# zyc-123/InstanceDiff

Measured on AMD Instinct MI355X. Metric: denoising steps/sec (256x256 bs16), higher is better.
Workload: dtype f32; 1 GPU; 256x256 1-ch synthetic, 1000-step reverse chain, batch 16 per GPU, 2 UNet fwd + reverse update per step; global_batch=16, parallelism=replicas x1 (no collective)

## Files before the change

### instancediff_amd/csrc/attention.hip

```cpp
#include <math.h>
#include <type_traits>
#include <stdlib.h>

#include "common.h"

namespace {

#define KAPPA(r) (((r) & 3) + 8 * ((r) >> 2))

template <int DH>
__global__ __launch_bounds__(256) void attn_self_kernel(const float* __restrict__ qkv, float* __restrict__ out, float* __restrict__ lse, int C,
                                                        int N, int heads, float scale) {
    constexpr int MB = DH / 32;
    constexpr int KT = DH * 32;
    constexpr int VT = DH * 33;
    constexpr int BUF = KT + VT + 3;
    constexpr int NV4 = DH * 32 / 4 / 256;
    extern __shared__ __attribute__((aligned(16))) float smem[];

    const int tid = threadIdx.x, lane = tid & 63, wave = tid >> 6, half = lane >> 5, l31 = lane & 31;
    const int b = blockIdx.y / heads, h = blockIdx.y % heads;
    const int q0 = (blockIdx.x * 4 + wave) * 32;
    const float* qb = qkv + (long long)b * 3 * C * N + (long long)(h * DH) * N;
    const float* kb = qb + (long long)C * N;
    const float* vb = qb + (long long)2 * C * N;

    float qreg[DH / 2];
    const int qi = q0 + l31;
#pragma unroll
    for (int s = 0; s < DH / 2; ++s) qreg[s] = qi < N ? qb[(long long)(2 * s + half) * N + qi] : 0.f;

    floatx16 O[MB];
#pragma unroll
    for (int m = 0; m < MB; ++m)
#pragma unroll
        for (int r = 0; r < 16; ++r) O[m][r] = 0.f;
    float mrun = -INFINITY, lrun = 0.f;

    const int nkb = (N + 31) / 32;
    floatx4 rk[NV4], rv[NV4];
    auto load_tile = [&](int kbi) {
        const int key0 = kbi * 32;
#pragma unroll
        for (int i = 0; i < NV4; ++i) {
            const int f = tid + i * 256;
            const int d = f >> 3, j4 = (f & 7) * 4;
            floatx4 kz = {0.f, 0.f, 0.f, 0.f}, vz = {0.f, 0.f, 0.f, 0.f};
            if (key0 + j4 + 3 < N) {
                kz = *reinterpret_cast<const floatx4*>(kb + (long long)d * N + key0 + j4);
                vz = *reinterpret_cast<const floatx4*>(vb + (long long)d * N + key0 + j4);
            } else {
                for (int e = 0; e < 4; ++e)
                    if (key0 + j4 + e < N) {
                        kz[e] = kb[(long long)d * N + key0 + j4 + e];
                        vz[e] = vb[(long long)d * N + key0 + j4 + e];
                    }
            }
            rk[i] = kz;
            rv[i] = vz;
        }
    };
    auto write_tile = [&](int buf) {
        float* kt = smem + buf * BUF;
        float* vt = kt + KT;
#pragma unroll
        for (int i = 0; i < NV4; ++i) {
            const int f = tid + i * 256;
            const int d = f >> 3, j4 = (f & 7) * 4;
#pragma unroll
            for (int e = 0; e < 4; ++e) {
                kt[d * 32 + j4 + e] = rk[i][e];
                vt[d * 33 + j4 + e] = rv[i][e];
            }
        }
    };

    load_tile(0);
    write_tile(0);
    __syncthreads();
    for (int kbi = 0; kbi < nkb; ++kbi) {
        const int buf = kbi & 1;
        if (kbi + 1 < nkb) load_tile(kbi + 1);
        const float* kt = smem + buf * BUF;
        const float* vt = kt + KT;
        floatx16 S;
#pragma unroll
        for (int r = 0; r < 16; ++r) S[r] = 0.f;
#pragma unroll
        for (int s = 0; s < DH / 2; ++s) S = __builtin_amdgcn_mfma_f32_32x32x2f32(kt[(2 * s + half) * 32 + l31], qreg[s], S, 0, 0, 0);
// ... 398 lines not shown
#pragma unroll
        for (int i = 0; i < NF4; ++i) {
            const int f = lane + i * 64;
            const int c = f >> 3, j4 = (f & 7) * 4;
            if (XCW % 8 != 0 && f >= XCW * 8) continue;
#pragma unroll
            for (int e = 0; e < 4; ++e) tile[c * 33 + j4 + e] = rt[i][e];
        }
    };

    if (kb_begin < kb_end) {
        load_tile(kb_begin);
        write_tile();
    }
    for (int kbi = kb_begin; kbi < kb_end; ++kbi) {
        if (kbi + 1 < kb_end) load_tile(kbi + 1);
        floatx16 S;
#pragma unroll
        for (int r = 0; r < 16; ++r) S[r] = 0.f;
#pragma unroll
        for (int t = 0; t < XCW / 2; ++t) S = __builtin_amdgcn_mfma_f32_32x32x2f32(tile[(2 * t + half) * 33 + l31], qreg[t], S, 0, 0, 0);
#pragma unroll
        for (int r = 0; r < 16; ++r) xch[(wave * 16 + r) * 64 + lane] = S[r];
        __syncthreads();
        const int key0 = kbi * 32 + 4 * half;
        float mx = -INFINITY;
#pragma unroll
        for (int r = 0; r < 16; ++r) {
            float sv = xch[(0 * 16 + r) * 64 + lane] + xch[(1 * 16 + r) * 64 + lane] + xch[(2 * 16 + r) * 64 + lane] + xch[(3 * 16 + r) * 64 + lane];
            sv = (key0 + KAPPA(r) < N) ? sv * scale : -INFINITY;
            S[r] = sv;
            mx = fmaxf(mx, sv);
        }
        mx = fmaxf(mx, __shfl_xor(mx, 32, 64));
        const float mnew = fmaxf(mrun, mx);
        const float alpha = __expf(mrun - mnew);
        float ps = 0.f;
#pragma unroll
        for (int r = 0; r < 16; ++r) {
            const float p = __expf(S[r] - mnew);
            S[r] = p;
            ps += p;
        }
        lrun = lrun * alpha + ps;
        mrun = mnew;
        if (__any(alpha != 1.f)) {
#pragma unroll
            for (int m = 0; m < XCB; ++m)
#pragma unroll
                for (int r = 0; r < 16; ++r) O[m][r] *= alpha;
        }
#pragma unroll
        for (int r = 0; r < 16; ++r)
#pragma unroll
            for (int m = 0; m < XCB; ++m)
                O[m] = __builtin_amdgcn_mfma_f32_32x32x2f32(tile[(m * 32 + l31) * 33 + KAPPA(r) + 4 * half], S[r], O[m], 0, 0, 0);
        if (kbi + 1 < kb_end) write_tile();
        __syncthreads();
    }
    float* wp = ws + ((long long)b * nsplit + sp) * (XCM + 2) * 32;
    const float l = lrun + __shfl_xor(lrun, 32, 64);
#pragma unroll
    for (int m = 0; m < XCB; ++m)
#pragma unroll
        for (int r = 0; r < 16; ++r) {
            const int cl = m * 32 + KAPPA(r) + 4 * half;
            if (cl < XCW) wp[(c0 + cl) * 32 + l31] = O[m][r];
        }
    if (wave == 0 && half == 0) {
        wp[XCM * 32 + l31] = mrun;
        wp[(XCM + 1) * 32 + l31] = l;
    }
}
template <int XCW>
__global__ __launch_bounds__(256) void smm_xattn_kernel(const float* __restrict__ qf, const float* __restrict__ mem, float* __restrict__ ws,
                                                        int rows, int N, int nsplit, int kps, float scale) {
    smm_xattn_body<XCW>(qf, mem, ws, rows, N, nsplit, kps, scale, blockIdx.y, blockIdx.x);
}

template <int CM>
__device__ __forceinline__ void smm_xattn_w_body(const float* __restrict__ qf, const float* __restrict__ mem, float* __restrict__ ws, int rows, int N,
                                                 int nsplit, int kps, float scale, const int b, const int sp) {
    constexpr int CB = (CM + 31) / 32;
    constexpr int TILE = CB * 32 * 33;
    constexpr int NF4 = (CM * 8 + 63) / 64;
    extern __shared__ __attribute__((aligned(16))) float smem[];
    const int tid = threadIdx.x, lane = tid & 63, wave = tid >> 6, half = lane >> 5, l31 = lane & 31;
    float* tile = smem + wave * TILE;
    const float* memb = mem + (long long)b * CM * N;
    for (int i = lane; i < TILE; i += 64) tile[i] = 0.f;

    float qreg[CM / 2];
#pragma unroll
    for (int t = 0; t < CM / 2; ++t) qreg[t] = l31 < rows ? qf[((long long)b * rows + l31) * CM + 2 * t + half] : 0.f;
    floatx16 O[CB];
#pragma unroll
    for (int m = 0; m < CB; ++m)
#pragma unroll
        for (int r = 0; r < 16; ++r) O[m][r] = 0.f;
    float mrun = -INFINITY, lrun = 0.f;

    const int nkb = (N + 31) / 32;
    const int kb_begin = sp * kps + wave;
    const int kb_end = min(nkb, sp * kps + kps);
    floatx4 rt[NF4];
    auto load_tile = [&](int kbi) {
        const int key0 = kbi * 32;
#pragma unroll
        for (int i = 0; i < NF4; ++i) {
            const int f = lane + i * 64;
            const int c = f >> 3, j4 = (f & 7) * 4;
            floatx4 z = {0.f, 0.f, 0.f, 0.f};
            if ((CM * 8) % 64 != 0 && f >= CM * 8) {
            } else if (key0 + j4 + 3 < N)
                z = *reinterpret_cast<const floatx4*>(memb + (long long)c * N + key0 + j4);
            else
                for (int e = 0; e < 4; ++e)
                    if (key0 + j4 + e < N) z[e] = memb[(long long)c * N + key0 + j4 + e];
            rt[i] = z;
        }
    };
    auto write_tile = [&]() {
#pragma unroll
        for (int i = 0; i < NF4; ++i) {
            const int f = lane + i * 64;
            const int c = f >> 3, j4 = (f & 7) * 4;
            if ((CM * 8) % 64 != 0 && f >= CM * 8) continue;
#pragma unroll
            for (int e = 0; e < 4; ++e) tile[c * 33 + j4 + e] = rt[i][e];
        }
    };
    if (kb_begin < kb_end) load_tile(kb_begin);
    for (int kbi = kb_begin; kbi < kb_end; kbi += 4) {
        write_tile();
        if (kbi + 4 < kb_end) load_tile(kbi + 4);
        floatx16 S;
#pragma unroll
        for (int r = 0; r < 16; ++r) S[r] = 0.f;
#pragma unroll
        for (int t = 0; t < CM / 2; ++t) S = __builtin_amdgcn_mfma_f32_32x32x2f32(tile[(2 * t + half) * 33 + l31], qreg[t], S, 0, 0, 0);
        const int key0 = kbi * 32 + 4 * half;
        float mx = -INFINITY;
#pragma unroll
        for (int r = 0; r < 16; ++r) {
            const float sv = (key0 + KAPPA(r) < N) ? S[r] * scale : -INFINITY;
            S[r] = sv;
            mx = fmaxf(mx, sv);
        }
        mx = fmaxf(mx, __shfl_xor(mx, 32, 64));
        const float mnew = fmaxf(mrun, mx);
        const float alpha = __expf(mrun - mnew);
        float ps = 0.f;
#pragma unroll
        for (int r = 0; r < 16; ++r) {
            const float p = __expf(S[r] - mnew);
            S[r] = p;
            ps += p;
        }
        lrun = lrun * alpha + ps;
        mrun = mnew;
        if (__any(alpha != 1.f)) {
#pragma unroll
            for (int m = 0; m < CB; ++m)
#pragma unroll
                for (int r = 0; r < 16; ++r) O[m][r] *= alpha;
        }
#pragma unroll
        for (int r = 0; r < 16; ++r)
#pragma unroll
            for (int m = 0; m < CB; ++m)
                O[m] = __builtin_amdgcn_mfma_f32_32x32x2f32(tile[(m * 32 + l31) * 33 + KAPPA(r) + 4 * half], S[r], O[m], 0, 0, 0);
    }
    static_assert((CM + 2) * 32 <= TILE, "partial does not fit the tile area");
    const float l = lrun + __shfl_xor(lrun, 32, 64);
#pragma unroll
    for (int m = 0; m < CB; ++m)
#pragma unroll
        for (int r = 0; r < 16; ++r) {
            const int cl = m * 32 + KAPPA(r) + 4 * half;
            if (cl < CM) tile[cl * 32 + l31] = O[m][r];
        }
    if (half == 0) {
        tile[CM * 32 + l31] = mrun;
        tile[(CM + 1) * 32 + l31] = l;
    }
    __syncthreads();
    float* wp = ws + ((long long)b * nsplit + sp) * (CM + 2) * 32;
    for (int i = tid; i < CM * 32; i += 256) {
        const int row = i & 31;
        float M = -INFINITY;
#pragma unroll
        for (int w = 0; w < 4; ++w) M = fmaxf(M, smem[w * TILE + CM * 32 + row]);
        float acc = 0.f;
#pragma unroll
        for (int w = 0; w < 4; ++w) {
            const float ms = smem[w * TILE + CM * 32 + row];
            acc += smem[w * TILE + i] * (ms == -INFINITY ? 0.f : __expf(ms - M));
        }
        wp[i] = acc;
    }
    if (tid < 32) {
        float M = -INFINITY, L = 0.f;
#pragma unroll
        for (int w = 0; w < 4; ++w) M = fmaxf(M, smem[w * TILE + CM * 32 + tid]);
#pragma unroll
        for (int w = 0; w < 4; ++w) {
            const float ms = smem[w * TILE + CM * 32 + tid];
            L += smem[w * TILE + (CM + 1) * 32 + tid] * (ms == -INFINITY ? 0.f : __expf(ms - M));
        }
        wp[CM * 32 + tid] = M;
        wp[(CM + 1) * 32 + tid] = L;
    }
}
template <int CM>
__global__ __launch_bounds__(256) void smm_xattn_w_kernel(const float* __restrict__ qf, const float* __restrict__ mem, float* __restrict__ ws, int rows,
                                                          int N, int nsplit, int kps, float scale) {
    smm_xattn_w_body<CM>(qf, mem, ws, rows, N, nsplit, kps, scale, blockIdx.y, blockIdx.x);
}

constexpr int CSL = 4;
__device__ __forceinline__ void smm_xattn_combine_body(const float* __restrict__ ws, float* __restrict__ o, int rows, int nsplit, int XCM,
                                                       float* __restrict__ lse, const int b, const int bx) {
    __shared__ float red[3][CSL][64];
    const int io = threadIdx.x & 63, sl = threadIdx.x >> 6;
    const int i = bx * 64 + io;
    const int c = i >> 5, row = i & 31;
    const bool live = i < XCM * 32 && row < rows;
    const long long ss = (long long)(XCM + 2) * 32;
    const float* wb = ws + (long long)b * nsplit * ss;
    float M = -INFINITY, L = 0.f, acc = 0.f;
    if (live) {
#pragma unroll 8
        for (int s = sl; s < nsplit; s += CSL) M = fmaxf(M, wb[s * ss + XCM * 32 + row]);
#pragma unroll 8
        for (int s = sl; s < nsplit; s += CSL) {
            const float* w = wb + s * ss;
            const float ms = w[XCM * 32 + row];
            const float f = ms == -INFINITY ? 0.f : __expf(ms - M);
            L += w[(XCM + 1) * 32 + row] * f;
            acc += w[c * 32 + row] * f;
        }
    }
    red[0][sl][io] = M, red[1][sl][io] = L, red[2][sl][io] = acc;
    __syncthreads();
    if (sl == 0 && live) {
        float Mt = red[0][0][io];
#pragma unroll
        for (int l = 1; l < CSL; ++l) Mt = fmaxf(Mt, red[0][l][io]);
        float Lt = 0.f, At = 0.f;
#pragma unroll
        for (int l = 0; l < CSL; ++l) {
            const float ml = red[0][l][io];
            const float f = ml == -INFINITY ? 0.f : __expf(ml - Mt);
            Lt += red[1][l][io] * f;
            At += red[2][l][io] * f;
        }
        o[((long long)b * rows + row) * XCM + c] = At / Lt;
        if (lse && c == 0) lse[(long long)b * rows + row] = Mt + __logf(Lt);
    }
}
__global__ __launch_bounds__(256) void smm_xattn_combine_kernel(const float* __restrict__ ws, float* __restrict__ o, int rows, int nsplit, int XCM,
                                                                float* __restrict__ lse) {
    smm_xattn_combine_body(ws, o, rows, nsplit, XCM, lse, blockIdx.y, blockIdx.x);
}

struct XattnGroups {
    idiff_xattn_group g[IDIFF_XATTN_MAX_GROUPS];
    int nsplit[IDIFF_XATTN_MAX_GROUPS], kps[IDIFF_XATTN_MAX_GROUPS], kind[IDIFF_XATTN_MAX_GROUPS];
};
__global__ __launch_bounds__(256) __attribute__((amdgpu_waves_per_eu(2))) void smm_xattn_grouped_kernel(const XattnGroups args, int rows, float scale) {
    const int z = blockIdx.z;
    const idiff_xattn_group& d = args.g[z];
    const int ns = args.nsplit[z], kps = args.kps[z];
    if ((int)blockIdx.x >= ns) return;
    switch (args.kind[z]) {
        case 0: smm_xattn_body<64>(d.qf, d.mem, d.ws, rows, d.N, ns, kps, scale, blockIdx.y, blockIdx.x); break;
        case 1: smm_xattn_body<34>(d.qf, d.mem, d.ws, rows, d.N, ns, kps, scale, blockIdx.y, blockIdx.x); break;
        case 2: smm_xattn_body<18>(d.qf, d.mem, d.ws, rows, d.N, ns, kps, scale, blockIdx.y, blockIdx.x); break;
        default: smm_xattn_w_body<72>(d.qf, d.mem, d.ws, rows, d.N, ns, kps, scale, blockIdx.y, blockIdx.x); break;
    }
}
__global__ __launch_bounds__(256) void smm_xattn_combine_grouped_kernel(const XattnGroups args, int rows) {
    const int z = blockIdx.z;
    const idiff_xattn_group& d = args.g[z];
    if ((int)blockIdx.x * 64 >= d.Cm * 32) return;
    smm_xattn_combine_body(d.ws, d.o, rows, args.nsplit[z], d.Cm, nullptr, blockIdx.y, blockIdx.x);
}

template <int XCW>
__global__ __launch_bounds__(256) void smm_xattn_bwd_kernel(const float* __restrict__ qf, const float* __restrict__ mem, const float* __restrict__ o,
                                                            const float* __restrict__ lse, const float* __restrict__ d_o, float* __restrict__ ws,
                                                            float* __restrict__ dmem, int rows, int N, int nsplit, int kps, float scale,
                                                            int accumulate) {
    constexpr int XCM = 4 * XCW, XCB = (XCW + 31) / 32, XTILE = XCB * 32 * 33, XP = XCM + 1, XREG = 2304;
    constexpr int NF4 = (XCW * 8 + 63) / 64;
    extern __shared__ __attribute__((aligned(16))) float smem[];
    float* tile = smem + (threadIdx.x >> 6) * XTILE;
    float* qL = smem + 4 * XTILE;
// ... 243 lines not shown
    else if (dh == 32)
        hipLaunchKernelGGL(attn_ctx_kernel<32>, grid, dim3(256), lds, st, q, k, v, out, C, N, M, scale);
    else if (dh == 64)
        hipLaunchKernelGGL(attn_ctx_kernel<64>, grid, dim3(256), lds, st, q, k, v, out, C, N, M, scale);
    else
        IDIFF_FAIL(IDIFF_E_UNSUPPORTED, "attn_ctx: head dim must be 16, 32 or 64 (got %d)", dh);
    IDIFF_CHECK_LAUNCH("attn_ctx_fwd");
    return IDIFF_OK;
}

extern "C" int idiff_attn_tokens_fwd(const float* q, const float* k, const float* v, float* out, int B, int Nq, int M, int C, int heads,
                                     float scale, int64_t ldq, int64_t ldkv, idiff_stream_t stream) {
    IDIFF_CHECK_ARG(q && k && v && out && B > 0 && Nq > 0 && C > 0 && heads > 0 && C % heads == 0, "attn_tokens: bad args");
    IDIFF_CHECK_ARG(M >= 1 && M <= 64, "attn_tokens: M must be in 1..64 (got %d)", M);
    IDIFF_CHECK_ARG(ldq >= C && ldkv >= C, "attn_tokens: row strides must be >= C");
    hipLaunchKernelGGL(attn_tokens_kernel, dim3(B * heads * Nq), dim3(64), 0, (hipStream_t)stream, q, k, v, out, Nq, M, C, heads, scale,
                       (long long)ldq, (long long)ldkv);
    IDIFF_CHECK_LAUNCH("attn_tokens_fwd");
    return IDIFF_OK;
}

extern "C" int idiff_attn_tokens_bwd(const float* q, const float* k, const float* v, const float* d_o, float* dq, float* dk, float* dv, int B, int Nq,
                                     int M, int C, int heads, float scale, int64_t ldq, int64_t ldkv, int64_t ldo, int64_t lddq, int64_t lddkv,
                                     idiff_stream_t stream) {
    IDIFF_CHECK_ARG(q && k && v && d_o && dq && dk && dv && B > 0 && C > 0 && heads > 0 && C % heads == 0, "attn_tokens_bwd: bad args");
    IDIFF_CHECK_ARG(Nq >= 1 && Nq <= ATB && M >= 1 && M <= ATB, "attn_tokens_bwd: Nq and M must be in 1..%d (got %d, %d)", ATB, Nq, M);
    IDIFF_CHECK_ARG(C / heads <= 64, "attn_tokens_bwd: head dim must be <= 64 (got %d)", C / heads);
    IDIFF_CHECK_ARG(ldq >= C && ldkv >= C && ldo >= C && lddq >= C && lddkv >= C, "attn_tokens_bwd: row strides must be >= C");
    hipLaunchKernelGGL(attn_tokens_bwd_kernel, dim3(B * heads), dim3(64), 0, (hipStream_t)stream, q, k, v, d_o, dq, dk, dv, Nq, M, C, heads, scale,
                       (long long)ldq, (long long)ldkv, (long long)ldo, (long long)lddq, (long long)lddkv);
    IDIFF_CHECK_LAUNCH("attn_tokens_bwd");
    return IDIFF_OK;
}

extern "C" int idiff_attn_tokens_grouped_fwd(const float* const* q, const float* const* k, const float* const* v, float* const* out, int ngroups,
                                             int B, int Nq, int M, int C, int heads, float scale, int64_t ldq, int64_t ldkv, idiff_stream_t stream) {
    IDIFF_CHECK_ARG(q && k && v && out && ngroups >= 1 && ngroups <= IDIFF_LINEAR_MAX_GROUPS, "attn_tokens_grouped: 1..%d groups", IDIFF_LINEAR_MAX_GROUPS);
    IDIFF_CHECK_ARG(B > 0 && Nq > 0 && C > 0 && heads > 0 && C % heads == 0, "attn_tokens_grouped: bad args");
    IDIFF_CHECK_ARG(M >= 1 && M <= 64, "attn_tokens_grouped: M must be in 1..64 (got %d)", M);
    IDIFF_CHECK_ARG(ldq >= C && ldkv >= C, "attn_tokens_grouped: row strides must be >= C");
    AttnTokGroups g;
    memset(&g, 0, sizeof(g));
    for (int i = 0; i < ngroups; ++i) {
        IDIFF_CHECK_ARG(q[i] && k[i] && v[i] && out[i], "attn_tokens_grouped: group %d: null pointer", i);
        g.q[i] = q[i], g.k[i] = k[i], g.v[i] = v[i], g.out[i] = out[i];
    }
    hipLaunchKernelGGL(attn_tokens_grouped_kernel, dim3(B * heads * Nq, ngroups), dim3(64), 0, (hipStream_t)stream, g, Nq, M, C, heads, scale,
                       (long long)ldq, (long long)ldkv);
    IDIFF_CHECK_LAUNCH("attn_tokens_grouped_fwd");
    return IDIFF_OK;
}

extern "C" int64_t idiff_smm_xattn_ws_floats(int B, int Nq, int heads, int Cm, int N) {
    (void)Nq;
    (void)heads;
    int ns, kps;
    smm_split(B, N, &ns, &kps);
    return (int64_t)B * ns * (Cm + 2) * 32;
}

static int smm_xattn_fwd_impl(const float* qf, const float* mem, float* o, float* lse, float* ws, int B, int Nq, int heads, int Cm, int N, float scale,
                              idiff_stream_t stream) {
    IDIFF_CHECK_ARG(qf && mem && o && ws && B > 0 && Nq > 0 && heads > 0 && N > 0, "smm_xattn: bad args");
    IDIFF_CHECK_ARG(Cm == 256 || Cm == 136 || Cm == 72, "smm_xattn: Cm must be 72, 136 or 256 (got %d)", Cm);
    IDIFF_CHECK_ARG(Nq * heads <= 32, "smm_xattn: Nq*heads must be <= 32 (got %d)", Nq * heads);
    IDIFF_CHECK_ARG(N % 4 == 0, "smm_xattn: N must be a multiple of 4");
    int ns, kps;
    smm_split(B, N, &ns, &kps);
    const int rows = Nq * heads;
    hipStream_t st = (hipStream_t)stream;
    const int xcb = (Cm / 4 + 31) / 32;
    const size_t lds = (size_t)(4 * xcb * 32 * 33 + 4 * 16 * 64) * sizeof(float);
    int ns_eff = ns;
    if (Cm == 256)
        hipLaunchKernelGGL(smm_xattn_kernel<64>, dim3(ns, B), dim3(256), lds, st, qf, mem, ws, rows, N, ns, kps, scale);
    else if (Cm == 136)
        hipLaunchKernelGGL(smm_xattn_kernel<34>, dim3(ns, B), dim3(256), lds, st, qf, mem, ws, rows, N, ns, kps, scale);
    else if (kps >= 4) {
        static const bool wform_off = [] {
            const char* e = getenv("IDIFF_XATTN_WFORM");
            return e && e[0] == '0';
        }();
        if (!wform_off) {
            const size_t ldsw = (size_t)4 * 3 * 32 * 33 * sizeof(float);
            hipLaunchKernelGGL(smm_xattn_w_kernel<72>, dim3(ns, B), dim3(256), ldsw, st, qf, mem, ws, rows, N, ns, kps, scale);
        } else {
            hipLaunchKernelGGL(smm_xattn_kernel<18>, dim3(ns, B), dim3(256), lds, st, qf, mem, ws, rows, N, ns, kps, scale);
        }
    } else
        hipLaunchKernelGGL(smm_xattn_kernel<18>, dim3(ns, B), dim3(256), lds, st, qf, mem, ws, rows, N, ns, kps, scale);
    IDIFF_CHECK_LAUNCH("smm_xattn_fwd");
    hipLaunchKernelGGL(smm_xattn_combine_kernel, dim3((32 * Cm + 63) / 64, B), dim3(256), 0, st, ws, o, rows, ns_eff, Cm, lse);
    IDIFF_CHECK_LAUNCH("smm_xattn_combine");
    return IDIFF_OK;
}

extern "C" int idiff_smm_xattn_grouped_fwd(const idiff_xattn_group* groups, int ngroups, int B, int Nq, int heads, float scale, idiff_stream_t stream) {
    IDIFF_CHECK_ARG(groups && ngroups >= 1 && ngroups <= IDIFF_XATTN_MAX_GROUPS, "smm_xattn_grouped: 1..%d groups", IDIFF_XATTN_MAX_GROUPS);
    IDIFF_CHECK_ARG(B > 0 && Nq > 0 && heads > 0 && Nq * heads <= 32, "smm_xattn_grouped: Nq*heads must be in 1..32 (got %d)", Nq * heads);
    XattnGroups args;
    memset(&args, 0, sizeof(args));
    int gx = 0, gc = 0;
    size_t lds = 0;
    for (int i = 0; i < ngroups; ++i) {
        const idiff_xattn_group& d = groups[i];
        IDIFF_CHECK_ARG(d.qf && d.mem && d.o && d.ws && d.N > 0 && d.N % 4 == 0, "smm_xattn_grouped: group %d: bad args", i);
        IDIFF_CHECK_ARG(d.Cm == 256 || d.Cm == 136 || d.Cm == 72, "smm_xattn_grouped: group %d: Cm must be 72, 136 or 256 (got %d)", i, d.Cm);
        args.g[i] = d;
        smm_split(B, d.N, &args.nsplit[i], &args.kps[i]);
        const int xcb = (d.Cm / 4 + 31) / 32;
        size_t l = (size_t)(4 * xcb * 32 * 33 + 4 * 16 * 64) * sizeof(float);
        if (d.Cm == 256) args.kind[i] = 0;
        else if (d.Cm == 136) args.kind[i] = 1;
        else if (args.kps[i] >= 4) args.kind[i] = 3, l = (size_t)4 * 3 * 32 * 33 * sizeof(float);
        else args.kind[i] = 2;
        lds = max(lds, l);
        gx = max(gx, args.nsplit[i]);
        gc = max(gc, (32 * d.Cm + 63) / 64);
    }
    hipStream_t st = (hipStream_t)stream;
    hipLaunchKernelGGL(smm_xattn_grouped_kernel, dim3(gx, B, ngroups), dim3(256), lds, st, args, Nq * heads, scale);
    IDIFF_CHECK_LAUNCH("smm_xattn_grouped_fwd");
    hipLaunchKernelGGL(smm_xattn_combine_grouped_kernel, dim3(gc, B, ngroups), dim3(256), 0, st, args, Nq * heads);
    IDIFF_CHECK_LAUNCH("smm_xattn_grouped_combine");
    return IDIFF_OK;
}

extern "C" int idiff_smm_xattn_fwd(const float* qf, const float* mem, float* o, float* ws, int B, int Nq, int heads, int Cm, int N, float scale,
                                   idiff_stream_t stream) {
    return smm_xattn_fwd_impl(qf, mem, o, nullptr, ws, B, Nq, heads, Cm, N, scale, stream);
}

extern "C" int idiff_smm_xattn_lse_fwd(const float* qf, const float* mem, float* o, float* lse, float* ws, int B, int rows, int N, float scale,
                                       idiff_stream_t stream) {
    IDIFF_CHECK_ARG(lse, "smm_xattn_lse_fwd: null lse");
    return smm_xattn_fwd_impl(qf, mem, o, lse, ws, B, rows, 1, 256, N, scale, stream);
}

extern "C" int idiff_smm_xattn_cm_lse_fwd(const float* qf, const float* mem, float* o, float* lse, float* ws, int B, int rows, int Cm, int N,
                                          float scale, idiff_stream_t stream) {
    IDIFF_CHECK_ARG(lse, "smm_xattn_cm_lse_fwd: null lse");
    return smm_xattn_fwd_impl(qf, mem, o, lse, ws, B, rows, 1, Cm, N, scale, stream);
}

static int smm_xattn_bwd_impl(const float* qf, const float* mem, const float* o, const float* lse, const float* d_o, float* dqf, float* dmem,
                              int accumulate, float* ws, int B, int rows, int Cm, int N, float scale, idiff_stream_t stream) {
    IDIFF_CHECK_ARG(qf && mem && o && lse && d_o && dqf && dmem && ws && B > 0 && N > 0, "smm_xattn_bwd: bad args");
    IDIFF_CHECK_ARG(rows >= 1 && rows <= 32, "smm_xattn_bwd: rows must be in 1..32 (got %d)", rows);
    IDIFF_CHECK_ARG(Cm == 256 || Cm == 72, "smm_xattn_bwd: Cm must be 72 or 256 (got %d)", Cm);
    IDIFF_CHECK_ARG(N % 4 == 0, "smm_xattn_bwd: N must be a multiple of 4");
    int ns, kps;
    smm_split(B, N, &ns, &kps);
    hipStream_t st = (hipStream_t)stream;
    const int xcb = (Cm / 4 + 31) / 32;
    const size_t lds = (size_t)(4 * xcb * 32 * 33 + 2 * 32 * (Cm + 1) + 4 * 2304 + 64) * sizeof(float);
    static bool attr[2] = {false, false};
    const int which = Cm == 256 ? 0 : 1;
    if (!attr[which]) {
        hipError_t e = Cm == 256 ? hipFuncSetAttribute(reinterpret_cast<const void*>(smm_xattn_bwd_kernel<64>), hipFuncAttributeMaxDynamicSharedMemorySize, (int)lds)
                                 : hipFuncSetAttribute(reinterpret_cast<const void*>(smm_xattn_bwd_kernel<18>), hipFuncAttributeMaxDynamicSharedMemorySize, (int)lds);
        if (e != hipSuccess) IDIFF_FAIL(IDIFF_E_HIP, "smm_xattn_bwd: hipFuncSetAttribute: %s", hipGetErrorString(e));
        attr[which] = true;
    }
    if (Cm == 256)
        hipLaunchKernelGGL(smm_xattn_bwd_kernel<64>, dim3(ns, B), dim3(256), lds, st, qf, mem, o, lse, d_o, ws, dmem, rows, N, ns, kps, scale, accumulate);
    else
        hipLaunchKernelGGL(smm_xattn_bwd_kernel<18>, dim3(ns, B), dim3(256), lds, st, qf, mem, o, lse, d_o, ws, dmem, rows, N, ns, kps, scale, accumulate);
    IDIFF_CHECK_LAUNCH("smm_xattn_bwd");
    hipLaunchKernelGGL(smm_xattn_bwd_combine_kernel, dim3((Cm * 32 + 255) / 256, B), dim3(256), 0, st, ws, dqf, rows, ns, Cm);
    IDIFF_CHECK_LAUNCH("smm_xattn_bwd_combine");
    return IDIFF_OK;
}

extern "C" int idiff_smm_xattn_bwd(const float* qf, const float* mem, const float* o, const float* lse, const float* d_o, float* dqf, float* dmem,
                                   int accumulate, float* ws, int B, int rows, int N, float scale, idiff_stream_t stream) {
    return smm_xattn_bwd_impl(qf, mem, o, lse, d_o, dqf, dmem, accumulate, ws, B, rows, 256, N, scale, stream);
}

extern "C" int idiff_smm_xattn_cm_bwd(const float* qf, const float* mem, const float* o, const float* lse, const float* d_o, float* dqf, float* dmem,
                                      int accumulate, float* ws, int B, int rows, int Cm, int N, float scale, idiff_stream_t stream) {
    return smm_xattn_bwd_impl(qf, mem, o, lse, d_o, dqf, dmem, accumulate, ws, B, rows, Cm, N, scale, stream);
}
```

### instancediff_amd/csrc/conv1x1_x3.hip

```cpp
#include <stdlib.h>

#include <type_traits>

#include "conv_args.h"

using idiff_detail::ConvArgs;

namespace {

typedef unsigned uintx4 __attribute__((ext_vector_type(4)));
typedef __bf16 bf16x8 __attribute__((ext_vector_type(8)));

constexpr int BM = 64, CKB = 32, NT = 256;
constexpr int B_ISTR = 1088;
constexpr int B_KGSTR = 4 * B_ISTR;
constexpr int B_PLSTR = 4 * B_KGSTR;
constexpr int B_BYTES = 3 * B_PLSTR;
constexpr int A_PLSTR = 4 * 64 * 16;
constexpr int A_BYTES = 3 * A_PLSTR;
constexpr int OLD = 256 + 4;
static_assert(32 * OLD * 4 <= B_BYTES, "epilogue tile must fit in the B planes");

__host__ __device__ constexpr unsigned hi16(unsigned u) { return u & 0xffff0000u; }

__device__ __forceinline__ unsigned pack_hi(unsigned odd, unsigned even) { return __builtin_amdgcn_perm(odd, even, 0x07060302u); }

__device__ __forceinline__ void split3(const float (&x)[8], uintx4& p1, uintx4& p2, uintx4& p3) {
    unsigned u1[8], u2[8], u3[8];
#pragma unroll
    for (int c = 0; c < 8; ++c) {
        u1[c] = __builtin_bit_cast(unsigned, x[c]);
        const float r1 = x[c] - __builtin_bit_cast(float, hi16(u1[c]));
        u2[c] = __builtin_bit_cast(unsigned, r1);
        const float r2 = r1 - __builtin_bit_cast(float, hi16(u2[c]));
        u3[c] = __builtin_bit_cast(unsigned, r2);
    }
    p1 = uintx4{pack_hi(u1[1], u1[0]), pack_hi(u1[3], u1[2]), pack_hi(u1[5], u1[4]), pack_hi(u1[7], u1[6])};
    p2 = uintx4{pack_hi(u2[1], u2[0]), pack_hi(u2[3], u2[2]), pack_hi(u2[5], u2[4]), pack_hi(u2[7], u2[6])};
    p3 = uintx4{pack_hi(u3[1], u3[0]), pack_hi(u3[3], u3[2]), pack_hi(u3[5], u3[4]), pack_hi(u3[7], u3[6])};
}

template <typename T>
__device__ __forceinline__ T* scalar_ptr(const T* p) {
    const unsigned long long v = reinterpret_cast<unsigned long long>(p);
    const unsigned lo = __builtin_amdgcn_readfirstlane((unsigned)v), hi = __builtin_amdgcn_readfirstlane((unsigned)(v >> 32));
    return reinterpret_cast<T*>(((unsigned long long)hi << 32) | lo);
}

__device__ __forceinline__ floatx4 mma(const uintx4& a, const uintx4& b, const floatx4& c) {
    return __builtin_amdgcn_mfma_f32_16x16x32_bf16(__builtin_bit_cast(bf16x8, a), __builtin_bit_cast(bf16x8, b), c, 0, 0, 0);
}

template <bool UNSH>
__global__ __launch_bounds__(NT) __attribute__((amdgpu_waves_per_eu(2, 2))) void conv1x1_x3_kernel(const ConvArgs a, const unsigned short* __restrict__ wx3) {
    extern __shared__ __attribute__((aligned(16))) unsigned char smem_raw[];
    unsigned char* const Bs = smem_raw;
    unsigned char* const As = smem_raw + B_BYTES;
    float* const econst = reinterpret_cast<float*>(smem_raw + B_BYTES + A_BYTES);

    const int tid = threadIdx.x;
    const int lane = tid & 63;
    const int wave = __builtin_amdgcn_readfirstlane(tid >> 6);
    const int n16 = lane & 15, kgl = lane >> 4;

    const unsigned logical = xcd_remap(blockIdx.x, a.total_wg);
    const int cob = logical % a.ncob;
    const int tile = (logical / a.ncob) % a.ntiles;
    const int b = logical / (a.ncob * a.ntiles);
    const int co0 = cob * BM;
    const long long HW = (long long)a.Hout * a.Wout;
    const long long pix0 = (long long)tile * 256;

    {
        const int which = tid >> 6, co = co0 + (tid & 63);
        float v = 0.f;
        if (which == 0 && a.bias) v = a.bias[co];
        if (which == 1 && a.vec) v = a.vec[(long long)b * a.Cout + co];
        if (which == 2 && a.aux) v = a.aux_a[(long long)b * a.Cout + co];
        if (which == 3 && a.aux) v = a.aux_b[(long long)b * a.Cout + co];
        econst[tid] = v;
    }

    const int q = lane, kg = wave;
    const int nchunks = (a.Cin + CKB - 1) / CKB;
    floatx4 xrA[8], xrB[8];
    uintx4 ar[3];
    constexpr int RSRC_FLAGS = 0x00020000;
    const float* const s0 = a.src0 + (long long)b * a.bs0 + (UNSH ? 0 : pix0);
    const float* const s1 = a.src1 ? a.src1 + (long long)b * a.bs1 + pix0 : s0;
    const long long HWin = (long long)a.Hin * a.Win;
    const int chstride_b = (int)((UNSH ? HWin : HW) * 4);
    int xoff = q * 16;
    if (UNSH) {
        const int p = (int)pix0 + 4 * q;
        const int oy = p / a.Wout, ox = p - oy * a.Wout;
        xoff = (2 * oy * a.Win + 2 * ox) * 4;
    }
    auto load_x = [&](floatx4 (&xr)[8], int cc) {
        const int ch0 = cc * CKB + kg * 8;
        const bool valid = ch0 < a.Cin;
        if (UNSH) {
            const float* const p = s0 + (long long)(valid ? (ch0 >> 2) : 0) * HWin;
            const __amdgpu_buffer_rsrc_t rs = __builtin_amdgcn_make_buffer_rsrc(scalar_ptr(p), 0, __builtin_amdgcn_readfirstlane(valid ? 0x7fffffff : 0), RSRC_FLAGS);
#pragma unroll
            for (int c = 0; c < 8; ++c)
                xr[c] = __builtin_bit_cast(floatx4, __builtin_amdgcn_raw_buffer_load_b128(rs, xoff, (c >> 2) * chstride_b + ((c >> 1) & 1) * a.Win * 4 + (c & 1) * 16, 0));
        } else {
            const bool second = ch0 >= a.C0v;
            const float* const p = (second ? s1 : s0) + (long long)(valid ? (second ? ch0 - a.C0v : ch0) : 0) * HW;
            const __amdgpu_buffer_rsrc_t rs = __builtin_amdgcn_make_buffer_rsrc(scalar_ptr(p), 0, __builtin_amdgcn_readfirstlane(valid ? 0x7fffffff : 0), RSRC_FLAGS);
#pragma unroll
            for (int c = 0; c < 8; ++c) xr[c] = __builtin_bit_cast(floatx4, __builtin_amdgcn_raw_buffer_load_b128(rs, xoff, c * chstride_b, 0));
        }
    };
    auto load_w = [&](int cc) {
        const bool valid = cc < nchunks;
        const unsigned short* const wsrc = wx3 + ((long long)(valid ? cc : 0) * a.ncob + cob) * (A_BYTES / 2);
        const __amdgpu_buffer_rsrc_t rs = __builtin_amdgcn_make_buffer_rsrc(scalar_ptr(wsrc), 0, __builtin_amdgcn_readfirstlane(valid ? A_BYTES : 0), RSRC_FLAGS);
#pragma unroll
        for (int i = 0; i < 3; ++i) ar[i] = __builtin_bit_cast(uintx4, __builtin_amdgcn_raw_buffer_load_b128(rs, tid * 16, i * NT * 16, 0));
    };
    unsigned char* const bw = Bs + kg * B_KGSTR + q * 16;
    auto stage = [&](const floatx4 (&xr)[8]) {
#pragma unroll
        for (int i = 0; i < 4; ++i) {
            float v[8];
#pragma unroll
            for (int c = 0; c < 8; ++c) {
                if (UNSH) {
                    const int px = 2 * i + (c & 1);
                    v[c] = xr[(c >> 1) * 2 + (px >> 2)][px & 3];
                } else {
                    v[c] = xr[c][i];
                }
            }
            uintx4 p1, p2, p3;
            split3(v, p1, p2, p3);
            *reinterpret_cast<uintx4*>(bw + i * B_ISTR) = p1;
            *reinterpret_cast<uintx4*>(bw + i * B_ISTR + B_PLSTR) = p2;
            *reinterpret_cast<uintx4*>(bw + i * B_ISTR + 2 * B_PLSTR) = p3;
        }
#pragma unroll
        for (int i = 0; i < 3; ++i) reinterpret_cast<uintx4*>(As)[tid + i * NT] = ar[i];
    };

    floatx4 acc[4][4];
#pragma unroll
    for (int mi = 0; mi < 4; ++mi)
#pragma unroll
        for (int j = 0; j < 4; ++j) acc[mi][j] = floatx4{0.f, 0.f, 0.f, 0.f};
    const unsigned char* const ard = As + kgl * 1024 + n16 * 16;
    const unsigned char* const brd = Bs + kgl * B_KGSTR + (n16 & 3) * B_ISTR + (16 * wave + (n16 >> 2)) * 16;

    auto chunk = [&](int cc, auto par_tag) {
        constexpr int PAR = decltype(par_tag)::value;
        floatx4(&xr)[8] = PAR ? xrB : xrA;
        __syncthreads();
        __builtin_amdgcn_sched_barrier(0);
        stage(xr);
        __syncthreads();
        load_w(cc + 1);
        load_x(xr, cc + 2);
        __builtin_amdgcn_sched_barrier(0);
#pragma unroll
        for (int mh = 0; mh < 2; ++mh) {
            uintx4 av[2][3];
#pragma unroll
            for (int m2 = 0; m2 < 2; ++m2)
#pragma unroll
                for (int p = 0; p < 3; ++p) av[m2][p] = *reinterpret_cast<const uintx4*>(ard + p * A_PLSTR + (2 * mh + m2) * 256);
            uintx4 bv[2][3];
#pragma unroll
            for (int p = 0; p < 3; ++p) bv[0][p] = *reinterpret_cast<const uintx4*>(brd + p * B_PLSTR);
#pragma unroll
            for (int j = 0; j < 4; ++j) {
                if (j + 1 < 4) {
#pragma unroll
                    for (int p = 0; p < 3; ++p) bv[(j + 1) & 1][p] = *reinterpret_cast<const uintx4*>(brd + p * B_PLSTR + (j + 1) * 64);
                }
                const uintx4(&bj)[3] = bv[j & 1];
#pragma unroll
                for (int m2 = 0; m2 < 2; ++m2) {
                    floatx4 c = acc[2 * mh + m2][j];
                    c = mma(av[m2][2], bj[0], c);
                    c = mma(av[m2][1], bj[1], c);
                    c = mma(av[m2][0], bj[2], c);
                    c = mma(av[m2][1], bj[0], c);
                    c = mma(av[m2][0], bj[1], c);
                    c = mma(av[m2][0], bj[0], c);
                    acc[2 * mh + m2][j] = c;
                }
            }
        }
    };
    load_x(xrA, 0);
    load_w(0);
    load_x(xrB, 1);
    int cc = 0;
    for (; cc + 1 < nchunks; cc += 2) {
        chunk(cc, std::integral_constant<int, 0>{});
        chunk(cc + 1, std::integral_constant<int, 1>{});
    }
    if (cc < nchunks) chunk(cc, std::integral_constant<int, 0>{});

    float* const ot = reinterpret_cast<float*>(Bs);
    float* const outb = a.out + (long long)b * a.obs;
    const float* const resb = a.res ? a.res + (long long)b * a.rbs : nullptr;
    const float* const auxb = a.aux ? a.aux + (long long)b * a.abs_ : nullptr;
    auto rows = [&](int mb, auto res_tag, auto aux_tag) {
        constexpr bool RES = decltype(res_tag)::value, AUX = decltype(aux_tag)::value;
        constexpr int STEPS = 32 * 64 / NT;
        floatx4 nres = {0.f, 0.f, 0.f, 0.f}, naux = {0.f, 0.f, 0.f, 0.f};
        auto fetch = [&](int i) {
            const int f = tid + i * NT;
            const int row = mb * 32 + (f >> 6), c4 = (f & 63) * 4;
            const long long o = (long long)(co0 + row) * HW + pix0 + c4;
            if (RES) nres = *reinterpret_cast<const floatx4*>(resb + o);
            if (AUX) naux = *reinterpret_cast<const floatx4*>(auxb + o);
        };
        fetch(0);
        __syncthreads();
#pragma unroll
        for (int mh = 0; mh < 2; ++mh)
#pragma unroll
            for (int j = 0; j < 4; ++j)
#pragma unroll
                for (int r = 0; r < 4; ++r)
                    ot[(mh * 16 + 4 * kgl + r) * OLD + 64 * wave + 16 * j + n16] = mb ? acc[2 + mh][j][r] : acc[mh][j][r];
        __syncthreads();
#pragma unroll
        for (int i = 0; i < STEPS; ++i) {
            const int f = tid + i * NT;
            const int lrow = f >> 6, row = mb * 32 + lrow, c4 = (f & 63) * 4;
            const floatx4 cres = nres, caux = naux;
            if (i + 1 < STEPS) fetch(i + 1);
            floatx4 v = *reinterpret_cast<const floatx4*>(ot + lrow * OLD + c4);
            const float add = econst[row] + econst[BM + row];
            v = floatx4{v.x + add, v.y + add, v.z + add, v.w + add};
            if (RES) v = floatx4{v.x + cres.x, v.y + cres.y, v.z + cres.z, v.w + cres.w};
            if (AUX) {
                const float aa = econst[2 * BM + row], ab = econst[3 * BM + row];
                v = floatx4{v.x + silu_fast(aa * caux.x + ab), v.y + silu_fast(aa * caux.y + ab), v.z + silu_fast(aa * caux.z + ab),
                            v.w + silu_fast(aa * caux.w + ab)};
            }
            *reinterpret_cast<floatx4*>(outb + (long long)(co0 + row) * HW + pix0 + c4) = v;
        }
    };
    auto halves = [&](auto res_tag, auto aux_tag) {
        rows(0, res_tag, aux_tag);
        rows(1, res_tag, aux_tag);
    };
    if (resb) {
        if (auxb) halves(std::true_type{}, std::true_type{});
        else halves(std::true_type{}, std::false_type{});
    } else {
        if (auxb) halves(std::false_type{}, std::true_type{});
        else halves(std::false_type{}, std::false_type{});
    }
}

__global__ void pack_x3_kernel(const float* __restrict__ w, uintx4* __restrict__ out, int Cout, int Cin, int ncob, long long npieces) {
    for (long long i = blockIdx.x * (long long)blockDim.x + threadIdx.x; i < npieces; i += (long long)gridDim.x * blockDim.x) {
        const int co_l = i & 63;
        const int kg = (i >> 6) & 3;
        const int plane = (int)((i >> 8) % 3);
        const long long blk = i / 768;
        const int cob = (int)(blk % ncob), cc = (int)(blk / ncob);
        const int co = cob * 64 + co_l;
        float x[8];
#pragma unroll
        for (int e = 0; e < 8; ++e) {
            const int ci = cc * CKB + kg * 8 + e;
            x[e] = (co < Cout && ci < Cin) ? w[(long long)co * Cin + ci] : 0.f;
// ... 51 lines not shown
```

Before: 43.53 steps/s.

## Emulate FP32 cross-attention with split-BF16 MFMA using transposed LDS reads

The wide-memory cross-attention kernel (CM=72) now splits Q, K/V tiles and softmax probabilities into three BF16 planes and accumulates with six 32x32x16 BF16 MFMAs, replacing the slow 32x32x2 f32 MFMA. K tiles are stored in LDS as BF16 plane images and read transposed with ds_read_tr16. The split/mma6 helpers are shared with the conv kernel through a new header. The change adds a waves_per_eu hint and simplifies tail loads by clamping the address. The cost is extra split arithmetic and a reordered LDS layout, with accuracy close to FP32.

```diff
diff --git a/instancediff_amd/csrc/attention.hip b/instancediff_amd/csrc/attention.hip
--- a/instancediff_amd/csrc/attention.hip
+++ b/instancediff_amd/csrc/attention.hip
@@ -3,8 +3,14 @@
 #include <stdlib.h>
 
 #include "common.h"
+#include "split_bf16.h"
 
 namespace {
+
+using idiff_split::mma6;
+using idiff_split::split3;
+using idiff_split::uintx2;
+using idiff_split::uintx4;
 
 #define KAPPA(r) (((r) & 3) + 8 * ((r) >> 2))
 
@@ -569,17 +575,32 @@
 __device__ __forceinline__ void smm_xattn_w_body(const float* __restrict__ qf, const float* __restrict__ mem, float* __restrict__ ws, int rows, int N,
                                                  int nsplit, int kps, float scale, const int b, const int sp) {
     constexpr int CB = (CM + 31) / 32;
-    constexpr int TILE = CB * 32 * 33;
-    constexpr int NF4 = (CM * 8 + 63) / 64;
+    constexpr int KS = (CM + 15) / 16;
+    constexpr int VROW = 32 + 4;
+    constexpr int PLANE = (CM + 1) * VROW;
+    constexpr int TILE = 3 * PLANE / 2;
+    constexpr int NF4 = CM * 8 / 64;
+    static_assert(CM % 8 == 0 && PLANE % 4 == 0, "whole 16-byte loads per lane, 8-byte aligned slice images");
+    typedef short shortx4 __attribute__((ext_vector_type(4)));
+    typedef shortx4 __attribute__((address_space(3))) lds_shortx4;
     extern __shared__ __attribute__((aligned(16))) float smem[];
-    const int tid = threadIdx.x, lane = tid & 63, wave = tid >> 6, half = lane >> 5, l31 = lane & 31;
+    const int tid = threadIdx.x, lane = tid & 63, wave = __builtin_amdgcn_readfirstlane(tid >> 6), half = lane >> 5, l31 = lane & 31;
     float* tile = smem + wave * TILE;
+    unsigned short* const img = reinterpret_cast<unsigned short*>(tile);
     const float* memb = mem + (long long)b * CM * N;
     for (int i = lane; i < TILE; i += 64) tile[i] = 0.f;
 
-    float qreg[CM / 2];
-#pragma unroll
-    for (int t = 0; t < CM / 2; ++t) qreg[t] = l31 < rows ? qf[((long long)b * rows + l31) * CM + 2 * t + half] : 0.f;
+    uintx4 qp[KS][3];
+#pragma unroll
+    for (int s = 0; s < KS; ++s) {
+        float x[8];
+#pragma unroll
+        for (int e = 0; e < 8; ++e) {
+            const int c = 16 * s + 8 * half + e;
+            x[e] = (l31 < rows && c < CM) ? qf[((long long)b * rows + l31) * CM + c] : 0.f;
+        }
+        split3(x, qp[s][0], qp[s][1], qp[s][2]);
+    }
     floatx16 O[CB];
 #pragma unroll
     for (int m = 0; m < CB; ++m)
@@ -597,14 +618,9 @@
         for (int i = 0; i < NF4; ++i) {
             const int f = lane + i * 64;
             const int c = f >> 3, j4 = (f & 7) * 4;
-            floatx4 z = {0.f, 0.f, 0.f, 0.f};
-            if ((CM * 8) % 64 != 0 && f >= CM * 8) {
-            } else if (key0 + j4 + 3 < N)
-                z = *reinterpret_cast<const floatx4*>(memb + (long long)c * N + key0 + j4);
-            else
-                for (int e = 0; e < 4; ++e)
-                    if (key0 + j4 + e < N) z[e] = memb[(long long)c * N + key0 + j4 + e];
-            rt[i] = z;
+            const bool ok = key0 + j4 < N;
+            const floatx4 z = *reinterpret_cast<const floatx4*>(memb + (long long)c * N + (ok ? key0 + j4 : 0));
+            rt[i] = ok ? z : floatx4{0.f, 0.f, 0.f, 0.f};
         }
     };
     auto write_tile = [&]() {
@@ -612,10 +628,24 @@
         for (int i = 0; i < NF4; ++i) {
             const int f = lane + i * 64;
             const int c = f >> 3, j4 = (f & 7) * 4;
-            if ((CM * 8) % 64 != 0 && f >= CM * 8) continue;
-#pragma unroll
-            for (int e = 0; e < 4; ++e) tile[c * 33 + j4 + e] = rt[i][e];
-        }
+            uintx2 p[3];
+            split3(rt[i], p[0], p[1], p[2]);
+#pragma unroll
+            for (int pl = 0; pl < 3; ++pl) *reinterpret_cast<uintx2*>(img + pl * PLANE + c * VROW + j4) = p[pl];
+        }
+    };
+    const int trq = (lane >> 2) & 3, trk = 16 * ((lane >> 4) & 1) + 4 * (lane & 3);
+    auto s_operand = [&](int s, int pl) {
+        uintx4 k;
+#pragma unroll
+        for (int j = 0; j < 2; ++j) {
+            const int c0 = 16 * s + 8 * half + 4 * j;
+            const int row = c0 < CM ? c0 + trq : CM;
+            const shortx4 v = __builtin_amdgcn_ds_read_tr16_b64_v4i16((lds_shortx4*)(img + pl * PLANE + row * VROW + trk));
+            const uintx2 u = __builtin_bit_cast(uintx2, v);
+            k[2 * j] = u[0], k[2 * j + 1] = u[1];
+        }
+        return k;
     };
     if (kb_begin < kb_end) load_tile(kb_begin);
     for (int kbi = kb_begin; kbi < kb_end; kbi += 4) {
@@ -625,7 +655,12 @@
 #pragma unroll
         for (int r = 0; r < 16; ++r) S[r] = 0.f;
 #pragma unroll
-        for (int t = 0; t < CM / 2; ++t) S = __builtin_amdgcn_mfma_f32_32x32x2f32(tile[(2 * t + half) * 33 + l31], qreg[t], S, 0, 0, 0);
+        for (int s = 0; s < KS; ++s) {
+            uintx4 ka[3];
+#pragma unroll
+            for (int pl = 0; pl < 3; ++pl) ka[pl] = s_operand(s, pl);
+            S = mma6(ka, qp[s], S);
+        }
         const int key0 = kbi * 32 + 4 * half;
         float mx = -INFINITY;
 #pragma unroll
@@ -638,11 +673,16 @@
         const float mnew = fmaxf(mrun, mx);
         const float alpha = __expf(mrun - mnew);
         float ps = 0.f;
-#pragma unroll
-        for (int r = 0; r < 16; ++r) {
-            const float p = __expf(S[r] - mnew);
-            S[r] = p;
-            ps += p;
+        uintx4 pb[2][3];
+#pragma unroll
+        for (int t = 0; t < 2; ++t) {
+            float x[8];
+#pragma unroll
+            for (int e = 0; e < 8; ++e) {
+                x[e] = __expf(S[8 * t + e] - mnew);
+                ps += x[e];
+            }
+            split3(x, pb[t][0], pb[t][1], pb[t][2]);
         }
         lrun = lrun * alpha + ps;
         mrun = mnew;
@@ -653,10 +693,19 @@
                 for (int r = 0; r < 16; ++r) O[m][r] *= alpha;
         }
 #pragma unroll
-        for (int r = 0; r < 16; ++r)
-#pragma unroll
-            for (int m = 0; m < CB; ++m)
-                O[m] = __builtin_amdgcn_mfma_f32_32x32x2f32(tile[(m * 32 + l31) * 33 + KAPPA(r) + 4 * half], S[r], O[m], 0, 0, 0);
+        for (int t = 0; t < 2; ++t)
+#pragma unroll
+            for (int m = 0; m < CB; ++m) {
+                const int row = min(m * 32 + l31, CM);
+                uintx4 va[3];
+#pragma unroll
+                for (int pl = 0; pl < 3; ++pl) {
+                    const unsigned short* vr = img + pl * PLANE + row * VROW + 16 * t + 4 * half;
+                    const uintx2 lo = *reinterpret_cast<const uintx2*>(vr), hi = *reinterpret_cast<const uintx2*>(vr + 8);
+                    va[pl] = uintx4{lo[0], lo[1], hi[0], hi[1]};
+                }
+                O[m] = mma6(va, pb[t], O[m]);
+            }
     }
     static_assert((CM + 2) * 32 <= TILE, "partial does not fit the tile area");
     const float l = lrun + __shfl_xor(lrun, 32, 64);
@@ -700,7 +749,7 @@
     }
 }
 template <int CM>
-__global__ __launch_bounds__(256) void smm_xattn_w_kernel(const float* __restrict__ qf, const float* __restrict__ mem, float* __restrict__ ws, int rows,
+__global__ __launch_bounds__(256) __attribute__((amdgpu_waves_per_eu(2))) void smm_xattn_w_kernel(const float* __restrict__ qf, const float* __restrict__ mem, float* __restrict__ ws, int rows,
                                                           int N, int nsplit, int kps, float scale) {
     smm_xattn_w_body<CM>(qf, mem, ws, rows, N, nsplit, kps, scale, blockIdx.y, blockIdx.x);
 }
@@ -1110,7 +1159,7 @@
             return e && e[0] == '0';
         }();
         if (!wform_off) {
-            const size_t ldsw = (size_t)4 * 3 * 32 * 33 * sizeof(float);
+            const size_t ldsw = (size_t)4 * 3 * (72 + 1) * (32 + 4) * sizeof(uint16_t);
             hipLaunchKernelGGL(smm_xattn_w_kernel<72>, dim3(ns, B), dim3(256), ldsw, st, qf, mem, ws, rows, N, ns, kps, scale);
         } else {
             hipLaunchKernelGGL(smm_xattn_kernel<18>, dim3(ns, B), dim3(256), lds, st, qf, mem, ws, rows, N, ns, kps, scale);
@@ -1140,7 +1189,7 @@
         size_t l = (size_t)(4 * xcb * 32 * 33 + 4 * 16 * 64) * sizeof(float);
         if (d.Cm == 256) args.kind[i] = 0;
         else if (d.Cm == 136) args.kind[i] = 1;
-        else if (args.kps[i] >= 4) args.kind[i] = 3, l = (size_t)4 * 3 * 32 * 33 * sizeof(float);
+        else if (args.kps[i] >= 4) args.kind[i] = 3, l = (size_t)4 * 3 * (72 + 1) * (32 + 4) * sizeof(uint16_t);
         else args.kind[i] = 2;
         lds = max(lds, l);
         gx = max(gx, args.nsplit[i]);
diff --git a/instancediff_amd/csrc/conv1x1_x3.hip b/instancediff_amd/csrc/conv1x1_x3.hip
--- a/instancediff_amd/csrc/conv1x1_x3.hip
+++ b/instancediff_amd/csrc/conv1x1_x3.hip
@@ -3,13 +3,14 @@
 #include <type_traits>
 
 #include "conv_args.h"
+#include "split_bf16.h"
 
 using idiff_detail::ConvArgs;
+using idiff_split::mma6;
+using idiff_split::split3;
+using idiff_split::uintx4;
 
 namespace {
-
-typedef unsigned uintx4 __attribute__((ext_vector_type(4)));
-typedef __bf16 bf16x8 __attribute__((ext_vector_type(8)));
 
 constexpr int BM = 64, CKB = 32, NT = 256;
 constexpr int B_ISTR = 1088;
@@ -21,34 +22,11 @@
 constexpr int OLD = 256 + 4;
 static_assert(32 * OLD * 4 <= B_BYTES, "epilogue tile must fit in the B planes");
 
-__host__ __device__ constexpr unsigned hi16(unsigned u) { return u & 0xffff0000u; }
-
-__device__ __forceinline__ unsigned pack_hi(unsigned odd, unsigned even) { return __builtin_amdgcn_perm(odd, even, 0x07060302u); }
-
-__device__ __forceinline__ void split3(const float (&x)[8], uintx4& p1, uintx4& p2, uintx4& p3) {
-    unsigned u1[8], u2[8], u3[8];
-#pragma unroll
-    for (int c = 0; c < 8; ++c) {
-        u1[c] = __builtin_bit_cast(unsigned, x[c]);
-        const float r1 = x[c] - __builtin_bit_cast(float, hi16(u1[c]));
-        u2[c] = __builtin_bit_cast(unsigned, r1);
-        const float r2 = r1 - __builtin_bit_cast(float, hi16(u2[c]));
-        u3[c] = __builtin_bit_cast(unsigned, r2);
-    }
-    p1 = uintx4{pack_hi(u1[1], u1[0]), pack_hi(u1[3], u1[2]), pack_hi(u1[5], u1[4]), pack_hi(u1[7], u1[6])};
-    p2 = uintx4{pack_hi(u2[1], u2[0]), pack_hi(u2[3], u2[2]), pack_hi(u2[5], u2[4]), pack_hi(u2[7], u2[6])};
-    p3 = uintx4{pack_hi(u3[1], u3[0]), pack_hi(u3[3], u3[2]), pack_hi(u3[5], u3[4]), pack_hi(u3[7], u3[6])};
-}
-
 template <typename T>
 __device__ __forceinline__ T* scalar_ptr(const T* p) {
     const unsigned long long v = reinterpret_cast<unsigned long long>(p);
     const unsigned lo = __builtin_amdgcn_readfirstlane((unsigned)v), hi = __builtin_amdgcn_readfirstlane((unsigned)(v >> 32));
     return reinterpret_cast<T*>(((unsigned long long)hi << 32) | lo);
-}
-
-__device__ __forceinline__ floatx4 mma(const uintx4& a, const uintx4& b, const floatx4& c) {
-    return __builtin_amdgcn_mfma_f32_16x16x32_bf16(__builtin_bit_cast(bf16x8, a), __builtin_bit_cast(bf16x8, b), c, 0, 0, 0);
 }
 
 template <bool UNSH>
@@ -181,14 +159,7 @@
                 const uintx4(&bj)[3] = bv[j & 1];
 #pragma unroll
                 for (int m2 = 0; m2 < 2; ++m2) {
-                    floatx4 c = acc[2 * mh + m2][j];
-                    c = mma(av[m2][2], bj[0], c);
-                    c = mma(av[m2][1], bj[1], c);
-                    c = mma(av[m2][0], bj[2], c);
-                    c = mma(av[m2][1], bj[0], c);
-                    c = mma(av[m2][0], bj[1], c);
-                    c = mma(av[m2][0], bj[0], c);
-                    acc[2 * mh + m2][j] = c;
+                    acc[2 * mh + m2][j] = mma6(av[m2], bj, acc[2 * mh + m2][j]);
                 }
             }
         }
diff --git a/instancediff_amd/csrc/split_bf16.h b/instancediff_amd/csrc/split_bf16.h
--- /dev/null
+++ b/instancediff_amd/csrc/split_bf16.h
@@ -0,0 +1,63 @@
+#pragma once
+#include "common.h"
+
+namespace idiff_split {
+
+typedef unsigned uintx2 __attribute__((ext_vector_type(2)));
+typedef unsigned uintx4 __attribute__((ext_vector_type(4)));
+typedef __bf16 bf16x8 __attribute__((ext_vector_type(8)));
+
+__host__ __device__ constexpr unsigned hi16(unsigned u) { return u & 0xffff0000u; }
+
+__device__ __forceinline__ unsigned pack_hi(unsigned odd, unsigned even) { return __builtin_amdgcn_perm(odd, even, 0x07060302u); }
+
+__device__ __forceinline__ void split3(const float (&x)[8], uintx4& p1, uintx4& p2, uintx4& p3) {
+    unsigned u1[8], u2[8], u3[8];
+#pragma unroll
+    for (int c = 0; c < 8; ++c) {
+        u1[c] = __builtin_bit_cast(unsigned, x[c]);
+        const float r1 = x[c] - __builtin_bit_cast(float, hi16(u1[c]));
+        u2[c] = __builtin_bit_cast(unsigned, r1);
+        const float r2 = r1 - __builtin_bit_cast(float, hi16(u2[c]));
+        u3[c] = __builtin_bit_cast(unsigned, r2);
+    }
+    p1 = uintx4{pack_hi(u1[1], u1[0]), pack_hi(u1[3], u1[2]), pack_hi(u1[5], u1[4]), pack_hi(u1[7], u1[6])};
+    p2 = uintx4{pack_hi(u2[1], u2[0]), pack_hi(u2[3], u2[2]), pack_hi(u2[5], u2[4]), pack_hi(u2[7], u2[6])};
+    p3 = uintx4{pack_hi(u3[1], u3[0]), pack_hi(u3[3], u3[2]), pack_hi(u3[5], u3[4]), pack_hi(u3[7], u3[6])};
+}
+
+__device__ __forceinline__ void split3(const floatx4& x, uintx2& p1, uintx2& p2, uintx2& p3) {
+    unsigned u1[4], u2[4], u3[4];
+#pragma unroll
+    for (int c = 0; c < 4; ++c) {
+        const float xc = x[c];
+        u1[c] = __builtin_bit_cast(unsigned, xc);
+        const float r1 = xc - __builtin_bit_cast(float, hi16(u1[c]));
+        u2[c] = __builtin_bit_cast(unsigned, r1);
+        const float r2 = r1 - __builtin_bit_cast(float, hi16(u2[c]));
+        u3[c] = __builtin_bit_cast(unsigned, r2);
+    }
+    p1 = uintx2{pack_hi(u1[1], u1[0]), pack_hi(u1[3], u1[2])};
+    p2 = uintx2{pack_hi(u2[1], u2[0]), pack_hi(u2[3], u2[2])};
+    p3 = uintx2{pack_hi(u3[1], u3[0]), pack_hi(u3[3], u3[2])};
+}
+
+__device__ __forceinline__ floatx4 mma(const uintx4& a, const uintx4& b, const floatx4& c) {
+    return __builtin_amdgcn_mfma_f32_16x16x32_bf16(__builtin_bit_cast(bf16x8, a), __builtin_bit_cast(bf16x8, b), c, 0, 0, 0);
+}
+__device__ __forceinline__ floatx16 mma(const uintx4& a, const uintx4& b, const floatx16& c) {
+    return __builtin_amdgcn_mfma_f32_32x32x16_bf16(__builtin_bit_cast(bf16x8, a), __builtin_bit_cast(bf16x8, b), c, 0, 0, 0);
+}
+
+template <typename ACC>
+__device__ __forceinline__ ACC mma6(const uintx4 (&a)[3], const uintx4 (&b)[3], ACC c) {
+    c = mma(a[2], b[0], c);
+    c = mma(a[1], b[1], c);
+    c = mma(a[0], b[2], c);
+    c = mma(a[1], b[0], c);
+    c = mma(a[0], b[1], c);
+    c = mma(a[0], b[0], c);
+    return c;
+}
+
+}
```

Result: no change. 43.79 steps/s, median of 6 (+0.6%).
